# anihcsam/OpenGaussian

Measured on NVIDIA B200. Metric: fwd+bwd frames/sec @1M Gaussians 1080p, higher is better.
Workload: dtype f32

## Files before the change

opengaussian_b200/csrc/binning.cu:

```cuda
#include "common.cuh"

namespace ogs {

int radix_sort_pairs_u32(uint32_t* k0, uint32_t* k1, uint32_t* v0, uint32_t* v1, const uint32_t* n_ptr, uint64_t capacity,
                         int begin_bit, int end_bit, void* scratch, cudaStream_t s, int* result_in_second, uint32_t* n_valid);
int tile_sort_pairs_u16(uint16_t* k0, uint16_t* k1, uint32_t* v0, uint32_t* v1, const uint32_t* n_ptr, uint64_t capacity,
                        int bits, void* scratch, cudaStream_t s);
size_t tile_sort_scratch_bytes(uint64_t capacity);
void tile_sort_plan(int bits, int* passes, int* bits0);
uint32_t* tile_sort_pass0_counts(void* scratch);
size_t radix_scratch_bytes(uint64_t capacity, int passes);
size_t scan_scratch_bytes(int P);
int scan_gather(int P, const uint32_t* n_ptr, const uint32_t* order, const uint32_t* tiles, uint32_t* out, void* scratch,
                cudaStream_t s);

size_t depth_sort_temp_bytes(int P) {
    const size_t a = radix_scratch_bytes((uint64_t)P, 4) + 256, b = scan_scratch_bytes(P);
    return (a > b ? a : b);
}

size_t tile_sort_temp_bytes(int64_t cap) { return tile_sort_scratch_bytes((uint64_t)cap); }

__global__ void set_scalar_kernel(uint32_t* p, uint32_t v) { p[0] = v; p[1] = 0u; }

int depth_sort_and_scan(int P, const GeomPtrs& g, BinScratch& sc, cudaStream_t s, int debug) {
    uint32_t* n_ptr = (uint32_t*)((char*)sc.cub_temp + radix_scratch_bytes((uint64_t)P, 4));
    uint32_t* nvis = n_ptr + 1;
    int second = 0;
    set_scalar_kernel<<<1, 1, 0, s>>>(n_ptr, (uint32_t)P);
    int rc = radix_sort_pairs_u32(sc.dkeys_in, sc.dkeys_out, sc.dvals_in, sc.dvals_out, n_ptr, (uint64_t)P, 0, 32,
                                  sc.cub_temp, s, &second, nvis);
    if (rc) return rc;
    if (!second) {
        uint32_t* t = sc.dkeys_in; sc.dkeys_in = sc.dkeys_out; sc.dkeys_out = t;
        t = sc.dvals_in; sc.dvals_in = sc.dvals_out; sc.dvals_out = t;
    }
    sc.nvis_ptr = nvis;
    rc = scan_gather(P, nvis, sc.dvals_out, g.tiles, sc.offsets, sc.cub_temp, s);
    if (rc) return rc;
    OGS_KERNEL_CHECK("depth_sort_and_scan", debug, s);
    return 0;
}

__device__ __forceinline__ int imin_(int a, int b) { return a < b ? a : b; }
__device__ __forceinline__ int imax_(int a, int b) { return a > b ? a : b; }

#define EMIT_CHUNK 4096
__global__ void __launch_bounds__(256) emit_kernel(int P_cap, const uint32_t* __restrict__ nvis_ptr, int gx, int gy,
                                                   const uint32_t* __restrict__ n_ptr, uint32_t cap,
                                                   const uint32_t* __restrict__ order, const uint32_t* __restrict__ offsets,
                                                   const float4* __restrict__ rec0, const float4* __restrict__ rec1,
                                                   uint16_t* __restrict__ tkeys, uint32_t* __restrict__ tvals,
                                                   int bits0, uint32_t* __restrict__ cnt0 ) {
    __shared__ uint32_t s_hist[256];
    __shared__ uint32_t s_start[256];
    __shared__ uint32_t s_g[256];
    __shared__ uint32_t s_rect[256];
    __shared__ uint32_t s_w[256];
    __shared__ uint32_t s_round_end;
    const int t = threadIdx.x;
    const uint32_t N = min(*n_ptr, cap);
    const int P = (int)min(*nvis_ptr, (uint32_t)P_cap);
    const uint32_t chunk_lo = blockIdx.x * (uint32_t)EMIT_CHUNK;
    const uint32_t dmask = (1u << bits0) - 1u;
    if (chunk_lo >= N) {
        if (t < (1 << bits0)) cnt0[(size_t)t * gridDim.x + blockIdx.x] = 0u;
        return;
    }
    s_hist[t] = 0;
    const uint32_t chunk_hi = min(N, chunk_lo + (uint32_t)EMIT_CHUNK);
    int lo = 0, hi = P;
    while (lo < hi) {
        const int step = (hi - lo + 31) >> 5;
        const int pos = lo + ((t & 31) + 1) * step - 1;
        const bool gt = pos >= hi || __ldg(offsets + pos) > chunk_lo;
        const unsigned m = __ballot_sync(0xffffffffu, gt);
        if (m == 0u) { lo = hi; break; }
        const int f = __ffs(m) - 1;
        hi = min(hi, lo + (f + 1) * step - 1);
        lo = lo + f * step;
    }
    for (int round_start = lo; round_start < P; round_start += 256) {
        const int slot = round_start + t;
        uint32_t start = 0xFFFFFFFFu, g = 0, rect = 0, rw = 1;
        if (slot < P) {
            start = (slot == 0) ? 0u : __ldg(offsets + slot - 1);
            if (start < chunk_hi) {
                g = order[slot];
                const float4 b = rec1[g];
                const int radius = __float_as_int(b.w);
                if (radius > 0) {
                    const float4 a = rec0[g];
                    const float r = (float)radius;
                    const int x0 = imin_(gx, imax_(0, (int)((a.x - r) / 16.0f)));
                    const int y0 = imin_(gy, imax_(0, (int)((a.y - r) / 16.0f)));
                    const int x1 = imin_(gx, imax_(0, (int)((a.x + r + 15.0f) / 16.0f)));
                    rect = (uint32_t)x0 | ((uint32_t)y0 << 16);
                    rw = (uint32_t)(x1 - x0);
                }
            }
        }
        const int last_slot = min(P, round_start + 256) - 1;
        if (slot == last_slot) s_round_end = min(chunk_hi, __ldg(offsets + slot));
        s_start[t] = start;
        s_g[t] = g;
        s_rect[t] = rect;
        s_w[t] = rw;
        __syncthreads();
        const uint32_t e_lo = max(chunk_lo, s_start[0]);
        const uint32_t e_hi = s_round_end;
        for (uint32_t e = e_lo + t; e < e_hi; e += 256) {
            int j = 0;
#pragma unroll
            for (int step = 128; step >= 1; step >>= 1)
                if (s_start[j + step] <= e) j += step;
            const uint32_t rc = s_rect[j];
            const uint32_t local = e - s_start[j];
            const uint32_t w = s_w[j];
            const uint32_t dy = local / w, dx = local - dy * w;
            const uint32_t key = ((rc >> 16) + dy) * gx + (rc & 0xFFFFu) + dx;
            tkeys[e] = (uint16_t)key;
            tvals[e] = s_g[j];
            atomicAdd(&s_hist[key & dmask], 1u);
        }
        __syncthreads();
        if (e_hi >= chunk_hi) break;
    }
    __syncthreads();
    if (t < (1 << bits0)) cnt0[(size_t)t * gridDim.x + blockIdx.x] = s_hist[t];
}

__global__ void __launch_bounds__(256) ranges_kernel(const uint32_t* __restrict__ n_ptr, uint32_t cap,
                                                     const uint16_t* __restrict__ tk, uint2* __restrict__ ranges) {
    const uint32_t N = min(*n_ptr, cap);
    const uint32_t i0 = (blockIdx.x * 256u + threadIdx.x) * 8u;
    if (i0 >= N) return;
    uint32_t k[8];
    if (i0 + 8 <= N) {
        const uint4 q = __ldg(reinterpret_cast<const uint4*>(tk + i0));
        k[0] = q.x & 0xFFFFu; k[1] = q.x >> 16; k[2] = q.y & 0xFFFFu; k[3] = q.y >> 16;
        k[4] = q.z & 0xFFFFu; k[5] = q.z >> 16; k[6] = q.w & 0xFFFFu; k[7] = q.w >> 16;
    } else {
#pragma unroll
        for (int j = 0; j < 8; j++) k[j] = (i0 + j < N) ? tk[i0 + j] : 0xFFFFFFFFu;
    }
    uint32_t prev = (i0 == 0) ? 0xFFFFFFFFu : tk[i0 - 1];
#pragma unroll
    for (int j = 0; j < 8; j++) {
        const uint32_t i = i0 + j;
        if (i < N) {
            if (k[j] != prev) {
                ranges[k[j]].x = i;
                if (i > 0) ranges[prev].y = i;
            }
            if (i == N - 1) ranges[k[j]].y = N;
            prev = k[j];
        }
    }
}

int emit_sort_ranges(int P, int W, int H, const uint32_t* n_ptr, int64_t cap, const GeomPtrs& g, BinScratch& sc,
                     uint16_t* tkeys_a, uint32_t* tvals_a, uint16_t* tkeys_b, uint32_t* point_list, uint2* ranges,
                     cudaStream_t s, int debug) {
    const int gx = (W + 15) / 16, gy = (H + 15) / 16;
    const int tiles = gx * gy;
    OGS_CUDA(cudaMemsetAsync(ranges, 0, (size_t)tiles * sizeof(uint2), s));
    if (cap <= 0) return 0;
    int bits = 0;
    while ((1 << bits) < tiles) bits++;
    if (bits == 0) bits = 1;
    int passes = 1, bits0 = bits;
    tile_sort_plan(bits, &passes, &bits0);
    uint16_t* k0 = tkeys_a; uint16_t* k1 = tkeys_b;
    uint32_t* v0 = passes == 2 ? point_list : tvals_a;
    uint32_t* v1 = passes == 2 ? tvals_a : point_list;
    prof_begin(PF_EMIT, s);
    emit_kernel<<<(unsigned)((cap + EMIT_CHUNK - 1) / EMIT_CHUNK), 256, 0, s>>>(P, sc.nvis_ptr, gx, gy, n_ptr, (uint32_t)cap, sc.dvals_out,
                                                                                sc.offsets, g.rec0, g.rec1, k0, v0, bits0,
                                                                                tile_sort_pass0_counts(sc.cub_temp));
    prof_end(PF_EMIT, s);
    OGS_KERNEL_CHECK("emit_kernel", debug, s);
    prof_begin(PF_TILE_SORT, s);
    const int rc = tile_sort_pairs_u16(k0, k1, v0, v1, n_ptr, (uint64_t)cap, bits, sc.cub_temp, s);
    prof_end(PF_TILE_SORT, s);
    if (rc) return rc;
    OGS_KERNEL_CHECK("tile_sort", debug, s);
    const uint16_t* sorted_keys = passes == 2 ? k0 : k1;
    ProfScope ps(PF_RANGES, s);
    ranges_kernel<<<(unsigned)((cap + 2047) / 2048), 256, 0, s>>>(n_ptr, (uint32_t)cap, sorted_keys, ranges);
    OGS_KERNEL_CHECK("ranges_kernel", debug, s);
    return 0;
}

}
```

opengaussian_b200/csrc/radix.cu:

```cuda
#include <stdlib.h>

#include "common.cuh"

namespace ogs {

#define RS_THREADS 256
#define RS_WARPS 8
#define RS_ITEMS 16
#define RS_TILE (RS_THREADS * RS_ITEMS)
#define RS_ITEMS_SMALL 16
#define RS_TILE_SMALL (RS_THREADS * RS_ITEMS_SMALL)
#define RS_RADIX 256
#define RS_FLAG_AGG 0x40000000u
#define RS_FLAG_INC 0x80000000u
#define RS_VAL_MASK 0x3FFFFFFFu
#ifndef RS_LB
#define RS_LB 32
#endif

struct RsPasses {
    int num;
    int shift[4];
    int bits[4];
};

template <typename KeyT>
__global__ void __launch_bounds__(RS_THREADS) rs_hist_kernel(const KeyT* __restrict__ keys, const uint32_t* __restrict__ n_ptr,
                                                             uint32_t cap, RsPasses ps, uint32_t* __restrict__ ghist ,
                                                             uint32_t* __restrict__ n_valid) {
    __shared__ uint32_t s_h[4 * RS_RADIX];
    for (int e = threadIdx.x; e < ps.num * RS_RADIX; e += RS_THREADS) s_h[e] = 0;
    __syncthreads();
    const uint32_t n = min(*n_ptr, cap);
    uint32_t ndrop = 0;
    auto count = [&](uint32_t k) {
        ndrop += (k == 0xFFFFFFFFu) ? 1u : 0u;
#pragma unroll
        for (int p = 0; p < 4; p++)
            if (p < ps.num) atomicAdd(&s_h[p * RS_RADIX + ((k >> ps.shift[p]) & ((1u << ps.bits[p]) - 1u))], 1u);
    };
    if (sizeof(KeyT) == 4) {
        const uint32_t n4 = n / 4;
        const uint4* k4 = reinterpret_cast<const uint4*>(keys);
        for (uint32_t i = blockIdx.x * RS_THREADS + threadIdx.x; i < n4; i += 2 * gridDim.x * RS_THREADS) {
            const uint32_t i2 = i + gridDim.x * RS_THREADS;
            const uint4 qa = __ldg(k4 + i);
            const uint4 qb = i2 < n4 ? __ldg(k4 + i2) : make_uint4(0, 0, 0, 0);
            count(qa.x); count(qa.y); count(qa.z); count(qa.w);
            if (i2 < n4) { count(qb.x); count(qb.y); count(qb.z); count(qb.w); }
        }
        if (blockIdx.x == 0 && threadIdx.x < (n & 3u)) count((uint32_t)keys[n4 * 4 + threadIdx.x]);
    } else {
        for (uint32_t i = blockIdx.x * RS_THREADS + threadIdx.x; i < n; i += gridDim.x * RS_THREADS) count((uint32_t)keys[i]);
    }
    __syncthreads();
    if (n_valid) {
        __shared__ uint32_t s_drop;
        if (threadIdx.x == 0) s_drop = 0;
        __syncthreads();
#pragma unroll
        for (int m = 16; m >= 1; m >>= 1) ndrop += __shfl_xor_sync(0xffffffffu, ndrop, m);
        if ((threadIdx.x & 31) == 0 && ndrop) atomicAdd(&s_drop, ndrop);
        __syncthreads();
        if ((int)threadIdx.x < ps.num) s_h[threadIdx.x * RS_RADIX + ((1u << ps.bits[threadIdx.x]) - 1u)] -= s_drop;
        if (threadIdx.x == 0) atomicAdd(n_valid, (blockIdx.x == 0 ? n : 0u) - s_drop);
        __syncthreads();
    }
    for (int e = threadIdx.x; e < ps.num * RS_RADIX; e += RS_THREADS)
        if (s_h[e]) atomicAdd(&ghist[e], s_h[e]);
}

#ifndef RS_MINB
#define RS_MINB 2
#endif
template <typename KeyT, bool LOOKBACK, int ITEMS, bool DROP = false>
__global__ void __launch_bounds__(RS_THREADS, RS_MINB) rs_pass_kernel(const KeyT* __restrict__ kin, KeyT* __restrict__ kout,
                                                             const uint32_t* __restrict__ vin, uint32_t* __restrict__ vout,
                                                             const uint32_t* __restrict__ n_ptr, uint32_t cap, int shift, int bits,
                                                             const uint32_t* __restrict__ ghist ,
                                                             uint32_t* tile_state, uint32_t* ticket, uint32_t ntiles) {
    constexpr int TILE = RS_THREADS * ITEMS;
    __shared__ uint32_t s_wh[RS_WARPS * RS_RADIX];
    __shared__ uint32_t s_dstart[RS_RADIX];
    __shared__ uint32_t s_gbase[RS_RADIX];
    __shared__ __align__(16) KeyT s_keys[TILE];
    __shared__ __align__(16) uint32_t s_vals[TILE];
    __shared__ uint32_t s_tile, s_tile_valid;

    const int tid = threadIdx.x, warp = tid >> 5, lane = tid & 31;
    if (LOOKBACK && tid == 0) s_tile = atomicAdd(ticket, 1u);
    for (int e = tid; e < RS_WARPS * RS_RADIX; e += RS_THREADS) s_wh[e] = 0;
    __syncthreads();
    const uint32_t tile = LOOKBACK ? s_tile : blockIdx.x;
    const uint32_t n = min(*n_ptr, cap);
    const uint32_t tile_start = tile * (uint32_t)TILE;
    if (tile_start >= n) return;
    const uint32_t tile_n = min((uint32_t)TILE, n - tile_start);
    const uint32_t dmask = (1u << bits) - 1u;

    const uint32_t wbase = tile_start + warp * (32 * ITEMS);
    uint32_t key[ITEMS];
    uint32_t rank[ITEMS];
    const uint32_t lt_mask = (1u << lane) - 1u;
    uint32_t* wh = s_wh + warp * RS_RADIX;
    uint32_t val[ITEMS];
    constexpr int NK = (int)(ITEMS * sizeof(KeyT) / 16), NV = ITEMS / 4;
    const bool whole = !LOOKBACK && NK > 0 && NK * 16 == (int)(ITEMS * sizeof(KeyT)) && (ITEMS % 4) == 0 && tile_n == (uint32_t)TILE &&
                       (((uintptr_t)(kin + tile_start) | (uintptr_t)(vin + tile_start)) & 15) == 0;
    if (whole) {
        const uint4* ksrc = reinterpret_cast<const uint4*>(kin + tile_start);
        const uint4* vsrc = reinterpret_cast<const uint4*>(vin + tile_start);
        uint4 qk[NK > 0 ? NK : 1], qv[NV > 0 ? NV : 1];
#pragma unroll
        for (int u = 0; u < NK; u++) qk[u] = __ldg(ksrc + tid + u * RS_THREADS);
#pragma unroll
        for (int u = 0; u < NV; u++) qv[u] = __ldg(vsrc + tid + u * RS_THREADS);
#pragma unroll
        for (int u = 0; u < NK; u++) reinterpret_cast<uint4*>(s_keys)[tid + u * RS_THREADS] = qk[u];
#pragma unroll
        for (int u = 0; u < NV; u++) reinterpret_cast<uint4*>(s_vals)[tid + u * RS_THREADS] = qv[u];
        __syncthreads();
        const int lbase = warp * (32 * ITEMS) + lane;
#pragma unroll
        for (int i = 0; i < ITEMS; i++) {
            key[i] = (uint32_t)s_keys[lbase + i * 32];
            val[i] = s_vals[lbase + i * 32];
        }
    } else {
#pragma unroll
        for (int i = 0; i < ITEMS; i++) {
            const uint32_t idx = wbase + i * 32 + lane;
            key[i] = idx < n ? (uint32_t)kin[idx] : 0xFFFFFFFFu;
        }
#pragma unroll
        for (int i = 0; i < ITEMS; i++) {
            const uint32_t idx = wbase + i * 32 + lane;
            val[i] = idx < n ? vin[idx] : 0u;
        }
    }
#pragma unroll
    for (int i = 0; i < ITEMS; i++) {
        const uint32_t idx = wbase + i * 32 + lane;
        const bool valid = idx < n && (!DROP || key[i] != 0xFFFFFFFFu);
        const uint32_t d = valid ? ((key[i] >> shift) & dmask) : 0xFFFFFFFFu;
        uint32_t peers = __ballot_sync(0xffffffffu, valid);
        if (!valid) peers = ~peers;
#pragma unroll
        for (int bb = 0; bb < 8; bb++) {
            if (bb < bits) {
                const bool bit = (d >> bb) & 1u;
                const uint32_t m = __ballot_sync(0xffffffffu, bit);
                peers &= bit ? m : ~m;
            }
        }
        const int leader = __ffs(peers) - 1;
        uint32_t pre = 0;
        if (valid && lane == leader) {
            pre = wh[d];
            wh[d] = pre + __popc(peers);
        }
        pre = __shfl_sync(0xffffffffu, pre, leader);
        rank[i] = pre + __popc(peers & lt_mask);
        __syncwarp();
    }
    __syncthreads();

    uint32_t count = 0;
    {
        const int d = tid;
#pragma unroll
        for (int w = 0; w < RS_WARPS; w++) {
            const uint32_t t = s_wh[w * RS_RADIX + d];
            s_wh[w * RS_RADIX + d] = count;
            count += t;
        }
    }
    __syncthreads();
    uint32_t dstart = 0, dbase = 0;
    {
        const uint32_t gtot = (LOOKBACK || tid < (1 << bits)) ? ghist[tid] : 0u;
        uint32_t a = count, b = gtot;
#pragma unroll
        for (int o = 1; o < 32; o <<= 1) {
            const uint32_t ta = __shfl_up_sync(0xffffffffu, a, o), tb = __shfl_up_sync(0xffffffffu, b, o);
            if (lane >= o) { a += ta; b += tb; }
        }
        __shared__ uint32_t s_wa[RS_WARPS], s_wb[RS_WARPS];
        if (lane == 31) { s_wa[warp] = a; s_wb[warp] = b; }
        __syncthreads();
        uint32_t oa = 0, ob = 0;
#pragma unroll
        for (int w = 0; w < RS_WARPS; w++)
            if (w < warp) { oa += s_wa[w]; ob += s_wb[w]; }
        dstart = oa + a - count;
        dbase = ob + b - gtot;
        if (DROP && tid == RS_THREADS - 1) s_tile_valid = dstart + count;
    }
    if (!LOOKBACK) {
        const int d = tid;
        const uint32_t excl = (d < (1 << bits)) ? tile_state[(size_t)d * ntiles + tile] : 0u;
        s_dstart[d] = dstart;
        s_gbase[d] = dbase + excl - dstart;
    } else {
        const int d = tid;
        volatile uint32_t* st = tile_state;
        uint32_t excl = 0;
        if (tile == 0) {
            st[(size_t)tile * RS_RADIX + d] = count | RS_FLAG_INC;
        } else {
            st[(size_t)tile * RS_RADIX + d] = count | RS_FLAG_AGG;
            __threadfence();
            int t = (int)tile - 1;
            while (t >= 0) {
                uint32_t v[RS_LB];
#pragma unroll
                for (int q = 0; q < RS_LB; q++)
                    v[q] = (t - q >= 0) ? st[(size_t)(t - q) * RS_RADIX + d] : RS_FLAG_INC;
#pragma unroll
                for (int q = 0; q < RS_LB; q++) {
                    if (v[q] & RS_FLAG_INC) { excl += v[q] & RS_VAL_MASK; t = -1; break; }
                    if (v[q] & RS_FLAG_AGG) { excl += v[q] & RS_VAL_MASK; t--; }
                    else break;
                }
            }
            st[(size_t)tile * RS_RADIX + d] = (excl + count) | RS_FLAG_INC;
        }
        s_dstart[d] = dstart;
        s_gbase[d] = dbase + excl - dstart;
    }
    __syncthreads();

#pragma unroll
    for (int i = 0; i < ITEMS; i++) {
        const uint32_t idx = wbase + i * 32 + lane;
        if (idx < n && (!DROP || key[i] != 0xFFFFFFFFu)) {
            const uint32_t d = (key[i] >> shift) & dmask;
            const uint32_t pos = s_dstart[d] + s_wh[warp * RS_RADIX + d] + rank[i];
            s_keys[pos] = (KeyT)key[i];
            s_vals[pos] = val[i];
        }
    }
    __syncthreads();
    const uint32_t tile_out = DROP ? s_tile_valid : tile_n;
    for (uint32_t j = tid; j < tile_out; j += RS_THREADS) {
        const KeyT k = s_keys[j];
        const uint32_t d = ((uint32_t)k >> shift) & dmask;
        const uint32_t dst = s_gbase[d] + j;
        kout[dst] = k;
        vout[dst] = s_vals[j];
    }
}

size_t radix_scratch_bytes(uint64_t capacity, int passes) {
    const size_t tiles = (size_t)((capacity + RS_THREADS * 4 - 1) / (RS_THREADS * 4)) + 1;
    return align_up((size_t)4 * RS_RADIX * 4, 256) + 256 + (size_t)passes * tiles * RS_RADIX * 4;
}

template <typename KeyT, int ITEMS>
static int radix_sort_pairs_t(KeyT* k0, KeyT* k1, uint32_t* v0, uint32_t* v1, const uint32_t* n_ptr, uint64_t capacity,
                              int begin_bit, int end_bit, void* scratch, cudaStream_t s, int* result_in_second,
                              uint32_t* n_valid = nullptr) {
    RsPasses ps;
    ps.num = 0;
    for (int b = begin_bit; b < end_bit && ps.num < 4; b += 8) {
        ps.shift[ps.num] = b;
        ps.bits[ps.num] = (end_bit - b) < 8 ? (end_bit - b) : 8;
        ps.num++;
    }
    if (ps.num >= 2 && ps.bits[ps.num - 1] < 8) {
        const int tot = ps.bits[ps.num - 2] + ps.bits[ps.num - 1];
        ps.bits[ps.num - 2] = (tot + 1) / 2;
        ps.shift[ps.num - 1] = ps.shift[ps.num - 2] + ps.bits[ps.num - 2];
        ps.bits[ps.num - 1] = tot - ps.bits[ps.num - 2];
    }
    constexpr int TILE = RS_THREADS * ITEMS;
    const size_t tiles = (size_t)((capacity + TILE - 1) / TILE) + 1;
    char* base = (char*)scratch;
    uint32_t* ghist = (uint32_t*)base;
    uint32_t* tickets = (uint32_t*)(base + align_up((size_t)4 * RS_RADIX * 4, 256));
    uint32_t* states = (uint32_t*)(base + align_up((size_t)4 * RS_RADIX * 4, 256) + 256);
    OGS_CUDA(cudaMemsetAsync(scratch, 0, align_up((size_t)4 * RS_RADIX * 4, 256) + 256 + (size_t)ps.num * tiles * RS_RADIX * 4, s));
    int hist_grid = (int)((capacity + RS_THREADS * 8 - 1) / (RS_THREADS * 8));
    if (hist_grid > OGS_NUM_SMS * 4) hist_grid = OGS_NUM_SMS * 4;
    if (hist_grid < 1) hist_grid = 1;
    rs_hist_kernel<KeyT><<<hist_grid, RS_THREADS, 0, s>>>(k0, n_ptr, (uint32_t)capacity, ps, ghist, n_valid);
    KeyT* ka = k0; KeyT* kb = k1;
    uint32_t* va = v0; uint32_t* vb = v1;
    const unsigned grid = (unsigned)((capacity + TILE - 1) / TILE);
    for (int p = 0; p < ps.num; p++) {
        if (n_valid && p == 0)
            rs_pass_kernel<KeyT, true, ITEMS, true><<<grid, RS_THREADS, 0, s>>>(ka, kb, va, vb, n_ptr, (uint32_t)capacity, ps.shift[p],
                                                                                ps.bits[p], ghist + p * RS_RADIX,
                                                                                states + (size_t)p * tiles * RS_RADIX, tickets + p, 0u);
        else
            rs_pass_kernel<KeyT, true, ITEMS><<<grid, RS_THREADS, 0, s>>>(ka, kb, va, vb, n_valid ? n_valid : n_ptr, (uint32_t)capacity,
                                                                          ps.shift[p], ps.bits[p], ghist + p * RS_RADIX,
                                                                          states + (size_t)p * tiles * RS_RADIX, tickets + p, 0u);
        KeyT* tk = ka; ka = kb; kb = tk;
        uint32_t* tv = va; va = vb; vb = tv;
    }
    *result_in_second = (ps.num & 1);
    cudaError_t e = cudaGetLastError();
    if (e != cudaSuccess) return cuda_fail(e, "radix_sort_pairs");
    return 0;
}

int radix_sort_pairs_u32(uint32_t* k0, uint32_t* k1, uint32_t* v0, uint32_t* v1, const uint32_t* n_ptr, uint64_t capacity,
                         int begin_bit, int end_bit, void* scratch, cudaStream_t s, int* result_in_second, uint32_t* n_valid) {
    static const int env_items = getenv("OGS_RS_ITEMS") ? atoi(getenv("OGS_RS_ITEMS")) : RS_ITEMS_SMALL;
    if (env_items == 4)
        return radix_sort_pairs_t<uint32_t, 4>(k0, k1, v0, v1, n_ptr, capacity, begin_bit, end_bit, scratch, s, result_in_second, n_valid);
    if (env_items == 8)
        return radix_sort_pairs_t<uint32_t, 8>(k0, k1, v0, v1, n_ptr, capacity, begin_bit, end_bit, scratch, s, result_in_second, n_valid);
    return radix_sort_pairs_t<uint32_t, 16>(k0, k1, v0, v1, n_ptr, capacity, begin_bit, end_bit, scratch, s, result_in_second,
                                            n_valid);
}
template <typename KeyT>
__global__ void __launch_bounds__(RS_THREADS) rs_tile_hist_kernel(const KeyT* __restrict__ keys, const uint32_t* __restrict__ n_ptr,
                                                                  uint32_t cap, int shift, int bits, uint32_t ntiles,
                                                                  uint32_t* __restrict__ cnt ) {
    __shared__ uint32_t s_h[RS_RADIX];
    const int tid = threadIdx.x;
    s_h[tid] = 0;
    __syncthreads();
    const uint32_t n = min(*n_ptr, cap);
    const uint32_t tile = blockIdx.x, start = tile * (uint32_t)RS_TILE;
    const uint32_t dmask = (1u << bits) - 1u;
    if (start < n) {
        const uint32_t end = min(n, start + (uint32_t)RS_TILE);
        if (sizeof(KeyT) == 2 && end - start == RS_TILE) {
            const uint4* src = reinterpret_cast<const uint4*>(keys + start);
            for (int e = tid; e < RS_TILE / 8; e += RS_THREADS) {
                const uint4 q = __ldg(src + e);
                const uint32_t w[4] = {q.x, q.y, q.z, q.w};
#pragma unroll
                for (int k = 0; k < 4; k++) {
                    atomicAdd(&s_h[((w[k] & 0xFFFFu) >> shift) & dmask], 1u);
                    atomicAdd(&s_h[((w[k] >> 16) >> shift) & dmask], 1u);
                }
            }
        } else {
            for (uint32_t i = start + tid; i < end; i += RS_THREADS) atomicAdd(&s_h[((uint32_t)keys[i] >> shift) & dmask], 1u);
        }
    }
    __syncthreads();
    if (tid < (1 << bits)) cnt[(size_t)tid * ntiles + tile] = s_h[tid];
}

__global__ void __launch_bounds__(RS_THREADS) rs_tile_scan_kernel(uint32_t* __restrict__ cnt, uint32_t ntiles,
                                                                  uint32_t* __restrict__ totals ) {
    __shared__ uint32_t s_w[RS_WARPS];
    __shared__ uint32_t s_carry;
    const int tid = threadIdx.x, warp = tid >> 5, lane = tid & 31;
    uint32_t* row = cnt + (size_t)blockIdx.x * ntiles;
    if (tid == 0) s_carry = 0;
    __syncthreads();
    for (uint32_t base = 0; base < ntiles; base += RS_THREADS * 4) {
        uint32_t v[4], sum = 0;
#pragma unroll
        for (int i = 0; i < 4; i++) {
            const uint32_t idx = base + tid * 4 + i;
            v[i] = idx < ntiles ? row[idx] : 0u;
            sum += v[i];
        }
        uint32_t a = sum;
#pragma unroll
        for (int o = 1; o < 32; o <<= 1) {
            const uint32_t t = __shfl_up_sync(0xffffffffu, a, o);
            if (lane >= o) a += t;
        }
        if (lane == 31) s_w[warp] = a;
        __syncthreads();
        uint32_t woff = 0, total = 0;
#pragma unroll
        for (int w = 0; w < RS_WARPS; w++) {
            if (w < warp) woff += s_w[w];
            total += s_w[w];
        }
        uint32_t run = s_carry + woff + (a - sum);
#pragma unroll
        for (int i = 0; i < 4; i++) {
            const uint32_t idx = base + tid * 4 + i;
            if (idx < ntiles) row[idx] = run;
            run += v[i];
        }
        __syncthreads();
        if (tid == 0) s_carry += total;
        __syncthreads();
    }
    if (tid == 0) totals[blockIdx.x] = s_carry;
}

static size_t tile_sort_ntiles(uint64_t capacity) { return (size_t)((capacity + RS_TILE - 1) / RS_TILE); }
size_t tile_sort_scratch_bytes(uint64_t capacity) {
    return align_up((size_t)2 * RS_RADIX * 4, 256) + (size_t)2 * RS_RADIX * tile_sort_ntiles(capacity) * 4;
}
void tile_sort_plan(int bits, int* passes, int* bits0) {
    if (bits <= 8) { *passes = 1; *bits0 = bits; }
    else { *passes = 2; *bits0 = (bits + 1) / 2; }
}
uint32_t* tile_sort_pass0_counts(void* scratch) { return (uint32_t*)((char*)scratch + align_up((size_t)2 * RS_RADIX * 4, 256)); }

int tile_sort_pairs_u16(uint16_t* k0, uint16_t* k1, uint32_t* v0, uint32_t* v1, const uint32_t* n_ptr, uint64_t capacity,
                        int bits, void* scratch, cudaStream_t s) {
    int passes, bits0;
    tile_sort_plan(bits, &passes, &bits0);
    const uint32_t ntiles = (uint32_t)tile_sort_ntiles(capacity);
    uint32_t* totals = (uint32_t*)scratch;
    uint32_t* cnt0 = tile_sort_pass0_counts(scratch);
    uint32_t* cnt1 = cnt0 + (size_t)RS_RADIX * ntiles;
    rs_tile_scan_kernel<<<1 << bits0, RS_THREADS, 0, s>>>(cnt0, ntiles, totals);
    rs_pass_kernel<uint16_t, false, RS_ITEMS><<<ntiles, RS_THREADS, 0, s>>>(k0, k1, v0, v1, n_ptr, (uint32_t)capacity, 0, bits0, totals,
                                                                  cnt0, nullptr, ntiles);
    if (passes == 2) {
        const int bits1 = bits - bits0;
        rs_tile_hist_kernel<uint16_t><<<ntiles, RS_THREADS, 0, s>>>(k1, n_ptr, (uint32_t)capacity, bits0, bits1, ntiles, cnt1);
        rs_tile_scan_kernel<<<1 << bits1, RS_THREADS, 0, s>>>(cnt1, ntiles, totals + RS_RADIX);
        rs_pass_kernel<uint16_t, false, RS_ITEMS><<<ntiles, RS_THREADS, 0, s>>>(k1, k0, v1, v0, n_ptr, (uint32_t)capacity, bits0, bits1,
                                                                      totals + RS_RADIX, cnt1, nullptr, ntiles);
    }
    cudaError_t e = cudaGetLastError();
    if (e != cudaSuccess) return cuda_fail(e, "tile_sort_pairs");
    return 0;
}

#define SC_THREADS 256
#define SC_ITEMS 8
#define SC_TILE (SC_THREADS * SC_ITEMS)

__global__ void __launch_bounds__(SC_THREADS) scan_gather_kernel(int P, const uint32_t* __restrict__ n_ptr,
                                                                 const uint32_t* __restrict__ order,
                                                                 const uint32_t* __restrict__ tiles, uint32_t* __restrict__ out,
                                                                 uint32_t* tile_state, uint32_t* ticket) {
    __shared__ uint32_t s_tile, s_warp[SC_THREADS / 32], s_excl;
    __shared__ unsigned long long s_excl64;
    const int tid = threadIdx.x, warp = tid >> 5, lane = tid & 31;
    if (tid == 0) s_tile = atomicAdd(ticket, 1u);
    __syncthreads();
    const uint32_t tile = s_tile;
    const uint32_t n = min(*n_ptr, (uint32_t)P);
    if (n == 0) {
        if (tile == 0 && tid == 0) { out[P] = 0u; out[P + 1] = 0u; }
        return;
    }
    if (tile * (uint32_t)SC_TILE >= n) return;
    const uint32_t base = tile * (uint32_t)SC_TILE + tid * SC_ITEMS;
    uint32_t v[SC_ITEMS];
    uint32_t sum = 0;
#pragma unroll
    for (int i = 0; i < SC_ITEMS; i++) {
        const uint32_t idx = base + i;
        v[i] = idx < n ? tiles[order[idx]] : 0u;
        sum += v[i];
        v[i] = sum;
    }
    uint32_t a = sum;
#pragma unroll
    for (int o = 1; o < 32; o <<= 1) {
        const uint32_t t = __shfl_up_sync(0xffffffffu, a, o);
        if (lane >= o) a += t;
    }
    if (lane == 31) s_warp[warp] = a;
    __syncthreads();
    uint32_t woff = 0, total = 0;
#pragma unroll
    for (int w = 0; w < SC_THREADS / 32; w++) {
        if (w < warp) woff += s_warp[w];
        total += s_warp[w];
    }
    {
        volatile uint32_t* st = tile_state;
        if (tid == 0) {
            st[tile] = total | RS_FLAG_AGG;
            s_excl = 0;
            s_excl64 = 0ull;
        }
        __syncthreads();
        uint32_t part = 0;
        unsigned long long part64 = 0ull;
        for (uint32_t t = tid; t < tile; t += SC_THREADS) {
            uint32_t x;
            do { x = st[t]; } while (!(x & RS_FLAG_AGG));
            part += x & RS_VAL_MASK;
            part64 += x & RS_VAL_MASK;
        }
#pragma unroll
        for (int m = 16; m >= 1; m >>= 1) {
            part += __shfl_xor_sync(0xffffffffu, part, m);
            part64 += __shfl_xor_sync(0xffffffffu, part64, m);
        }
        if (lane == 0 && part64) { atomicAdd(&s_excl, part); atomicAdd(&s_excl64, part64); }
    }
    __syncthreads();
    if (tid == 0 && tile == (n - 1) / (uint32_t)SC_TILE) {
        out[P] = s_excl + total;
        out[P + 1] = (s_excl64 + total > 0xFFFFFFFFull) ? 1u : 0u;
    }
    const uint32_t off = s_excl + woff + (a - sum);
#pragma unroll
    for (int i = 0; i < SC_ITEMS; i++) {
        const uint32_t idx = base + i;
        if (idx < n) out[idx] = off + v[i];
    }
}

size_t scan_scratch_bytes(int P) { return ((size_t)(P + SC_TILE - 1) / SC_TILE + 2) * 4 + 256; }

int scan_gather(int P, const uint32_t* n_ptr, const uint32_t* order, const uint32_t* tiles, uint32_t* out, void* scratch,
                cudaStream_t s) {
    if (P <= 0) return 0;
    const int ntiles = (P + SC_TILE - 1) / SC_TILE;
    OGS_CUDA(cudaMemsetAsync(scratch, 0, scan_scratch_bytes(P), s));
    uint32_t* ticket = (uint32_t*)scratch;
    uint32_t* states = (uint32_t*)((char*)scratch + 256);
    scan_gather_kernel<<<ntiles, SC_THREADS, 0, s>>>(P, n_ptr, order, tiles, out, states, ticket);
    cudaError_t e = cudaGetLastError();
    if (e != cudaSuccess) return cuda_fail(e, "scan_gather");
    return 0;
}

}
```

Measured before the change: 781.2.

## Fuse tile range computation into final tile-sort scatter pass

Removes the separate ranges kernel that re-read the sorted tile keys. The final radix pass now detects key-run boundaries in shared memory and records each tile's start and end with atomicMin, skipping the write of sorted keys. A small finish kernel then decodes the inverted end values and zeroes tiles that received no entries. The trade is added atomics in the scatter loop and reliance on runs inside a block mapping to contiguous destinations, in exchange for less global key traffic.

```diff
diff --git a/opengaussian_b200/csrc/binning.cu b/opengaussian_b200/csrc/binning.cu
--- a/opengaussian_b200/csrc/binning.cu
+++ b/opengaussian_b200/csrc/binning.cu
@@ -5,7 +5,7 @@
 int radix_sort_pairs_u32(uint32_t* k0, uint32_t* k1, uint32_t* v0, uint32_t* v1, const uint32_t* n_ptr, uint64_t capacity,
                          int begin_bit, int end_bit, void* scratch, cudaStream_t s, int* result_in_second, uint32_t* n_valid);
 int tile_sort_pairs_u16(uint16_t* k0, uint16_t* k1, uint32_t* v0, uint32_t* v1, const uint32_t* n_ptr, uint64_t capacity,
-                        int bits, void* scratch, cudaStream_t s);
+                        int bits, void* scratch, uint2* ranges, cudaStream_t s);
 size_t tile_sort_scratch_bytes(uint64_t capacity);
 void tile_sort_plan(int bits, int* passes, int* bits0);
 uint32_t* tile_sort_pass0_counts(void* scratch);
@@ -130,33 +130,11 @@
     if (t < (1 << bits0)) cnt0[(size_t)t * gridDim.x + blockIdx.x] = s_hist[t];
 }
 
-__global__ void __launch_bounds__(256) ranges_kernel(const uint32_t* __restrict__ n_ptr, uint32_t cap,
-                                                     const uint16_t* __restrict__ tk, uint2* __restrict__ ranges) {
-    const uint32_t N = min(*n_ptr, cap);
-    const uint32_t i0 = (blockIdx.x * 256u + threadIdx.x) * 8u;
-    if (i0 >= N) return;
-    uint32_t k[8];
-    if (i0 + 8 <= N) {
-        const uint4 q = __ldg(reinterpret_cast<const uint4*>(tk + i0));
-        k[0] = q.x & 0xFFFFu; k[1] = q.x >> 16; k[2] = q.y & 0xFFFFu; k[3] = q.y >> 16;
-        k[4] = q.z & 0xFFFFu; k[5] = q.z >> 16; k[6] = q.w & 0xFFFFu; k[7] = q.w >> 16;
-    } else {
-#pragma unroll
-        for (int j = 0; j < 8; j++) k[j] = (i0 + j < N) ? tk[i0 + j] : 0xFFFFFFFFu;
-    }
-    uint32_t prev = (i0 == 0) ? 0xFFFFFFFFu : tk[i0 - 1];
-#pragma unroll
-    for (int j = 0; j < 8; j++) {
-        const uint32_t i = i0 + j;
-        if (i < N) {
-            if (k[j] != prev) {
-                ranges[k[j]].x = i;
-                if (i > 0) ranges[prev].y = i;
-            }
-            if (i == N - 1) ranges[k[j]].y = N;
-            prev = k[j];
-        }
-    }
+__global__ void __launch_bounds__(256) tile_ranges_finish_kernel(int tiles, uint2* __restrict__ ranges) {
+    const int t = blockIdx.x * 256 + threadIdx.x;
+    if (t >= tiles) return;
+    const uint2 r = ranges[t];
+    ranges[t] = r.x == 0xFFFFFFFFu ? make_uint2(0u, 0u) : make_uint2(r.x, ~r.y);
 }
 
 int emit_sort_ranges(int P, int W, int H, const uint32_t* n_ptr, int64_t cap, const GeomPtrs& g, BinScratch& sc,
@@ -164,7 +142,7 @@
                      cudaStream_t s, int debug) {
     const int gx = (W + 15) / 16, gy = (H + 15) / 16;
     const int tiles = gx * gy;
-    OGS_CUDA(cudaMemsetAsync(ranges, 0, (size_t)tiles * sizeof(uint2), s));
+    OGS_CUDA(cudaMemsetAsync(ranges, cap > 0 ? 0xFF : 0, (size_t)tiles * sizeof(uint2), s));
     if (cap <= 0) return 0;
     int bits = 0;
     while ((1 << bits) < tiles) bits++;
@@ -181,14 +159,13 @@
     prof_end(PF_EMIT, s);
     OGS_KERNEL_CHECK("emit_kernel", debug, s);
     prof_begin(PF_TILE_SORT, s);
-    const int rc = tile_sort_pairs_u16(k0, k1, v0, v1, n_ptr, (uint64_t)cap, bits, sc.cub_temp, s);
+    const int rc = tile_sort_pairs_u16(k0, k1, v0, v1, n_ptr, (uint64_t)cap, bits, sc.cub_temp, ranges, s);
     prof_end(PF_TILE_SORT, s);
     if (rc) return rc;
     OGS_KERNEL_CHECK("tile_sort", debug, s);
-    const uint16_t* sorted_keys = passes == 2 ? k0 : k1;
     ProfScope ps(PF_RANGES, s);
-    ranges_kernel<<<(unsigned)((cap + 2047) / 2048), 256, 0, s>>>(n_ptr, (uint32_t)cap, sorted_keys, ranges);
-    OGS_KERNEL_CHECK("ranges_kernel", debug, s);
+    tile_ranges_finish_kernel<<<(unsigned)((tiles + 255) / 256), 256, 0, s>>>(tiles, ranges);
+    OGS_KERNEL_CHECK("tile_ranges_finish_kernel", debug, s);
     return 0;
 }
 
diff --git a/opengaussian_b200/csrc/radix.cu b/opengaussian_b200/csrc/radix.cu
--- a/opengaussian_b200/csrc/radix.cu
+++ b/opengaussian_b200/csrc/radix.cu
@@ -73,12 +73,13 @@
 #ifndef RS_MINB
 #define RS_MINB 2
 #endif
-template <typename KeyT, bool LOOKBACK, int ITEMS, bool DROP = false>
+template <typename KeyT, bool LOOKBACK, int ITEMS, bool DROP = false, bool RANGES = false>
 __global__ void __launch_bounds__(RS_THREADS, RS_MINB) rs_pass_kernel(const KeyT* __restrict__ kin, KeyT* __restrict__ kout,
                                                              const uint32_t* __restrict__ vin, uint32_t* __restrict__ vout,
                                                              const uint32_t* __restrict__ n_ptr, uint32_t cap, int shift, int bits,
                                                              const uint32_t* __restrict__ ghist ,
-                                                             uint32_t* tile_state, uint32_t* ticket, uint32_t ntiles) {
+                                                             uint32_t* tile_state, uint32_t* ticket, uint32_t ntiles,
+                                                             uint2* ranges) {
     constexpr int TILE = RS_THREADS * ITEMS;
     __shared__ uint32_t s_wh[RS_WARPS * RS_RADIX];
     __shared__ uint32_t s_dstart[RS_RADIX];
@@ -246,7 +247,12 @@
         const KeyT k = s_keys[j];
         const uint32_t d = ((uint32_t)k >> shift) & dmask;
         const uint32_t dst = s_gbase[d] + j;
-        kout[dst] = k;
+        if (RANGES) {
+            if (j == 0 || s_keys[j - 1] != k) atomicMin(&ranges[k].x, dst);
+            if (j + 1 == tile_out || s_keys[j + 1] != k) atomicMin(&ranges[k].y, ~(dst + 1u));
+        } else {
+            kout[dst] = k;
+        }
         vout[dst] = s_vals[j];
     }
 }
@@ -291,11 +297,11 @@
         if (n_valid && p == 0)
             rs_pass_kernel<KeyT, true, ITEMS, true><<<grid, RS_THREADS, 0, s>>>(ka, kb, va, vb, n_ptr, (uint32_t)capacity, ps.shift[p],
                                                                                 ps.bits[p], ghist + p * RS_RADIX,
-                                                                                states + (size_t)p * tiles * RS_RADIX, tickets + p, 0u);
+                                                                                states + (size_t)p * tiles * RS_RADIX, tickets + p, 0u, nullptr);
         else
             rs_pass_kernel<KeyT, true, ITEMS><<<grid, RS_THREADS, 0, s>>>(ka, kb, va, vb, n_valid ? n_valid : n_ptr, (uint32_t)capacity,
                                                                           ps.shift[p], ps.bits[p], ghist + p * RS_RADIX,
-                                                                          states + (size_t)p * tiles * RS_RADIX, tickets + p, 0u);
+                                                                          states + (size_t)p * tiles * RS_RADIX, tickets + p, 0u, nullptr);
         KeyT* tk = ka; ka = kb; kb = tk;
         uint32_t* tv = va; va = vb; vb = tv;
     }
@@ -402,7 +408,7 @@
 uint32_t* tile_sort_pass0_counts(void* scratch) { return (uint32_t*)((char*)scratch + align_up((size_t)2 * RS_RADIX * 4, 256)); }
 
 int tile_sort_pairs_u16(uint16_t* k0, uint16_t* k1, uint32_t* v0, uint32_t* v1, const uint32_t* n_ptr, uint64_t capacity,
-                        int bits, void* scratch, cudaStream_t s) {
+                        int bits, void* scratch, uint2* ranges, cudaStream_t s) {
     int passes, bits0;
     tile_sort_plan(bits, &passes, &bits0);
     const uint32_t ntiles = (uint32_t)tile_sort_ntiles(capacity);
@@ -410,14 +416,17 @@
     uint32_t* cnt0 = tile_sort_pass0_counts(scratch);
     uint32_t* cnt1 = cnt0 + (size_t)RS_RADIX * ntiles;
     rs_tile_scan_kernel<<<1 << bits0, RS_THREADS, 0, s>>>(cnt0, ntiles, totals);
-    rs_pass_kernel<uint16_t, false, RS_ITEMS><<<ntiles, RS_THREADS, 0, s>>>(k0, k1, v0, v1, n_ptr, (uint32_t)capacity, 0, bits0, totals,
-                                                                  cnt0, nullptr, ntiles);
-    if (passes == 2) {
+    if (passes == 1) {
+        rs_pass_kernel<uint16_t, false, RS_ITEMS, false, true><<<ntiles, RS_THREADS, 0, s>>>(
+            k0, k1, v0, v1, n_ptr, (uint32_t)capacity, 0, bits0, totals, cnt0, nullptr, ntiles, ranges);
+    } else {
+        rs_pass_kernel<uint16_t, false, RS_ITEMS><<<ntiles, RS_THREADS, 0, s>>>(k0, k1, v0, v1, n_ptr, (uint32_t)capacity, 0, bits0, totals,
+                                                                      cnt0, nullptr, ntiles, nullptr);
         const int bits1 = bits - bits0;
         rs_tile_hist_kernel<uint16_t><<<ntiles, RS_THREADS, 0, s>>>(k1, n_ptr, (uint32_t)capacity, bits0, bits1, ntiles, cnt1);
         rs_tile_scan_kernel<<<1 << bits1, RS_THREADS, 0, s>>>(cnt1, ntiles, totals + RS_RADIX);
-        rs_pass_kernel<uint16_t, false, RS_ITEMS><<<ntiles, RS_THREADS, 0, s>>>(k1, k0, v1, v0, n_ptr, (uint32_t)capacity, bits0, bits1,
-                                                                      totals + RS_RADIX, cnt1, nullptr, ntiles);
+        rs_pass_kernel<uint16_t, false, RS_ITEMS, false, true><<<ntiles, RS_THREADS, 0, s>>>(
+            k1, k0, v1, v0, n_ptr, (uint32_t)capacity, bits0, bits1, totals + RS_RADIX, cnt1, nullptr, ntiles, ranges);
     }
     cudaError_t e = cudaGetLastError();
     if (e != cudaSuccess) return cuda_fail(e, "tile_sort_pairs");
```

New measurement: 773.5, median of 6. 0.99x the previous value.
